# basecomplextech/spec

Hardware: AMD Instinct MI355X
Metric: Mmsg/s + GB/s decode (device-resident), 1M×256B batch, 1/2/4/8 MI355X (higher is better)
Workload: dtype u8; 1 GPU; flat16-decode; records_per_gpu=1048576, stream_bytes_per_gpu=267602339, parallelism=record-sharded x1, no collective, ranks=1, distinct_devices=1, rehearsal=False

## Files before the change

__graft_entry__.py:

```python
from __future__ import annotations

import os
import subprocess
import sys

ROOT = os.path.dirname(os.path.abspath(__file__))


def build() -> None:
    jobs = str(min(8, os.cpu_count() or 1))
    subprocess.run(["make", "-s", "-j", jobs, "-C", os.path.join(ROOT, "spec_amd", "csrc")], check=True)
    subprocess.run(["make", "-s", "-C", os.path.join(ROOT, "oracle")], check=True)
    if ROOT not in sys.path:
        sys.path.insert(0, ROOT)
    import spec_amd

    L = spec_amd.lib()
    import time

    t0 = time.time() - 1
    import ctypes as C

    L.spec_decode_flat_jit_compile(C.byref(spec_amd.FLAT16.c), 1 << 28, 1 << 20)
    from spec_amd import workload

    for sc in workload.bench_wide_schemas().values():
        L.spec_decode_flat_jit_compile(C.byref(sc.c), 1 << 28, 1 << 20)
    L.spec_decode_flat_jit_compile(C.byref(spec_amd.NESTED.item.c), 1 << 28, 1 << 20)
    L.spec_encode_flat_jit_compile(C.byref(spec_amd.FLAT16.c))
    L.spec_decode_nested_jit_compile(C.byref(spec_amd.NESTED.c))
    L.spec_encode_nested_jit_compile(C.byref(spec_amd.NESTED.c))
    from spec_amd.tree_catalog import precompiled_trees

    k = int(jobs)
    procs = [subprocess.Popen([sys.executable, "-c", f"import __graft_entry__ as g; g._compile_trees({i}, {k})"],
                              cwd=ROOT) for i in range(min(k, len(precompiled_trees())))]
    if any(p.wait() != 0 for p in procs):
        raise RuntimeError("schema-tree kernel compile failed")
    procs = [subprocess.Popen([sys.executable, "-c", f"import __graft_entry__ as g; g._compile_sweep({i}, {k})"],
                              cwd=ROOT) for i in range(k)]
    if any(p.wait() != 0 for p in procs):
        raise RuntimeError("shape-sweep kernel compile failed")
    cache = os.path.join(ROOT, "spec_amd", "jit_cache")
    for f in os.listdir(cache):
        if f.endswith(".co") and os.path.getmtime(os.path.join(cache, f)) < t0:
            os.remove(os.path.join(cache, f))


def _compile_trees(i: int, k: int) -> None:
    import ctypes as C

    import spec_amd
    from spec_amd.tree_catalog import precompiled_trees

    L = spec_amd.lib()
    for t in precompiled_trees()[i::k]:
        if L.spec_tree_jit_compile(C.byref(t.c)) <= 0:
            raise RuntimeError("schema-tree kernel compile failed")


def _compile_sweep(i: int, k: int) -> None:
    import ctypes as C

    import spec_amd
    from spec_amd import workload

    L = spec_amd.lib()
    sweep = workload.shape_sweep_schemas()
    work = [(2 if len(s) <= 9 else 24 if len(s) <= 25 else 58, name, "encode") for name, s in sweep.items() if len(s) <= 32]
    work += [(8, name, "decode") for name in sweep]
    shares = [[0, []] for _ in range(k)]
    for cost, name, prog in sorted(work, reverse=True):
        share = min(shares, key=lambda sh: sh[0])
        share[0] += cost
        share[1].append((name, prog))
    for name, prog in shares[i][1]:
        c = C.byref(sweep[name].c)
        size = L.spec_encode_flat_jit_compile(c) if prog == "encode" else L.spec_decode_flat_jit_compile(c, 1 << 28, 1 << 20)
        if size <= 0:
# ... 43 lines not shown
```

spec_amd/csrc/decode_core.hpp:

```cpp
#pragma once

#include "spec_device.hpp"

namespace spec {


struct FieldSet {
    uint8_t *status;
    uint64_t *errmask;
    uint64_t *present;
    uint32_t nfields;
    uint16_t tags[SPEC_KFIELDS];
    uint8_t kinds[SPEC_KFIELDS];
    uint16_t rank[SPEC_KFIELDS];
    void *cols[SPEC_KFIELDS];
};

struct DecodeArgs {
    const uint8_t *stream;
    uint64_t stream_len;
    const uint64_t *ends;
    uint64_t n;
    uint64_t r0;
    uint32_t head;
    uint32_t slab;
    uint32_t xcd;
    FieldSet f;
};

struct NestedArgs {
    const uint8_t *stream;
    uint64_t stream_len;
    const uint64_t *ends;
    uint64_t n;
    FieldSet outer;
    FieldSet item;
    uint32_t list_tag, list_rank;
    uint32_t *item_begin;
    uint64_t item_cap;
    uint64_t *group_base;
    uint64_t *total;
    uint32_t slab;
    uint32_t xcd;
    uint32_t head;
};

constexpr int DEC_WAVES = 4;
constexpr int SLAB_GUARD = 48;

constexpr int SLAB_MAX_CHUNKS = 40;
__host__ __device__ inline uint32_t decode_slab_bytes(double avg_record, double margin = 1.04) {
    const double span = avg_record * 64 * margin;
    int chunks = (int)(span / 1024.0) + 1;
    if (chunks > SLAB_MAX_CHUNKS) return 0;
    return (uint32_t)(SLAB_GUARD + chunks * 1024 + 32);
}
constexpr uint32_t NESTED_SLAB_MAX = 163840 / DEC_WAVES - 1024;
__host__ __device__ inline uint32_t nested_slab_bytes(double avg_record) {
    const uint32_t s = decode_slab_bytes(avg_record, 1.16);
    return s <= NESTED_SLAB_MAX ? s : 0u;
}


template <class Src>
__device__ __noinline__ long long table_search(const Src s, typename Src::pos_t tstart, uint32_t nent,
                                               bool big, uint32_t tag) {
    int left = 0, right = (int)nent - 1;
    while (left <= right) {
        int mid = (int)((unsigned)(left + right) >> 1);
        uint32_t cur;
        typename Src::pos_t p;
        if (big) {
            p = tstart + (typename Src::pos_t)mid * 6;
            cur = (s.u8(p) << 8) | s.u8(p + 1);
        } else {
            p = tstart + (typename Src::pos_t)mid * 3;
            cur = s.u8(p);
        }
        if (cur < tag) {
            left = mid + 1;
        } else if (cur > tag) {
            right = mid - 1;
        } else {
            if (big)
                return ((long long)s.u8(p + 2) << 24) | (s.u8(p + 3) << 16) | (s.u8(p + 4) << 8) | s.u8(p + 5);
            return (s.u8(p + 1) << 8) | s.u8(p + 2);
        }
    }
    return -1;
}


struct Val {
    uint64_t v0, v1, v2, v3;
};

struct Win {
    Tail t;
    uint64_t x0, x1, x2;
};

template <uint32_t KIND>
__host__ __device__ constexpr bool narrow_kind() {
    return KIND == K_BOOL || KIND == K_BYTE || KIND == K_INT16 || KIND == K_INT32 || KIND == K_UINT16 ||
// ... 248 lines not shown

template <bool LIST = false, class Src>
__device__ __forceinline__ Trailer parse_trailer(const Src &s, typename Src::pos_t rs, typename Src::pos_t re) {
    Trailer tr = {ST_OK, false, 0, 0, 0, 0};
    long long len = (long long)(re - rs);
    Tail t = load_tail(s, re);
    uint32_t type = (uint32_t)t.q0 & 0xff;
    const uint32_t T_SMALL = LIST ? T_LIST : T_MESSAGE, T_BIG = LIST ? T_BIG_LIST : T_BIG_MESSAGE;
    const uint32_t ESMALL = LIST ? 2u : 3u, EBIG = LIST ? 4u : 6u;
    if (type != T_SMALL && type != T_BIG) {
        tr.st = ST_INVALID_TYPE;
        return tr;
    }
    tr.big = type == T_BIG;
    uint64_t R = tail_r(t);
    uint32_t R2 = tail_r2(t);
    int m1, m2;
    uint32_t tsz = (uint32_t)rvarint<5>(R, R2, len - 1, m1);
    if (m1 < 0) {
        tr.st = ST_INVALID_TABLE_SIZE;
        return tr;
    }
    uint64_t Rs = (R >> (8 * m1)) | ((uint64_t)R2 << (64 - 8 * m1));
    uint32_t R2s = m1 >= 2 ? 0u : (R2 >> (8 * m1));
    uint32_t dsz = (uint32_t)rvarint<5>(Rs, R2s, len - 1 - m1, m2);
    if (m2 < 0) {
        tr.st = ST_INVALID_DATA_SIZE;
        return tr;
    }
    long long tend = (long long)(re - 1) - m1 - m2;
    long long ts = tend - (long long)tsz;
    if (ts < (long long)rs || tsz % (tr.big ? EBIG : ESMALL) != 0) {
        tr.st = ST_INVALID_TABLE;
        return tr;
    }
    if (ts - (long long)dsz < (long long)rs) {
        tr.st = ST_INVALID_DATA;
        return tr;
    }
    tr.tstart = ts;
    tr.dstart = ts - (long long)dsz;
    tr.dsize = dsz;
    tr.tsize = tsz;
    return tr;
}


struct RecInfo {
    Trailer tr;
    bool ok, sorted;
    uint32_t nent;
};

template <class Src>
__device__ __forceinline__ RecInfo rec_open(const Src &s, typename Src::pos_t rs, typename Src::pos_t re) {
    using pos_t = typename Src::pos_t;
    RecInfo ri;
    ri.tr = Trailer{ST_OK, false, 0, 0, 0, 0};
    ri.ok = false;
    ri.sorted = true;
    ri.nent = 0;
    if (re > rs) {
        ri.tr = parse_trailer(s, rs, re);
        ri.ok = ri.tr.st == ST_OK;
        ri.nent = ri.tr.tsize / (ri.tr.big ? 6u : 3u);
    }
    if (ri.ok) {
        const pos_t tstart = (pos_t)ri.tr.tstart;
        const uint32_t esz = ri.tr.big ? 6u : 3u;
        uint32_t prev = 0;
        bool sorted = true;
        for (uint32_t i0 = 0; i0 < ri.nent; i0 += 8) {
            uint32_t tg[8];
#pragma unroll
            for (int u = 0; u < 8; u++) {
                const uint32_t i = i0 + u < ri.nent ? i0 + u : ri.nent - 1;
                const pos_t p = tstart + (pos_t)(i * esz);
                const uint32_t b0 = s.u8(p), b1 = s.u8(p + 1);
                tg[u] = ri.tr.big ? ((b0 << 8) | b1) : b0;
            }
#pragma unroll
            for (int u = 0; u < 8; u++) {
                const uint32_t i = i0 + u;
                const bool in = i < ri.nent;
                sorted = sorted & !(in & (i > 0) & (tg[u] <= prev));
                prev = in ? tg[u] : prev;
            }
        }
        ri.sorted = sorted;
    }
    return ri;
}

template <class Src>
__device__ __forceinline__ long long rec_field_end(const Src &s, const RecInfo &ri, uint32_t tag, uint32_t k) {
    using pos_t = typename Src::pos_t;
    if (!ri.ok) return -1;
    const pos_t tstart = (pos_t)ri.tr.tstart;
    long long end = -1;
    bool hit = false;
    if (ri.sorted && k < ri.nent) {
        if (ri.tr.big) {
            pos_t p = tstart + (pos_t)k * 6;
            uint32_t tg = (s.u8(p) << 8) | s.u8(p + 1);
            if (tg == tag) {
                end = ((long long)s.u8(p + 2) << 24) | (s.u8(p + 3) << 16) | (s.u8(p + 4) << 8) | s.u8(p + 5);
                hit = true;
            }
        } else {
            pos_t p = tstart + (pos_t)k * 3;
            if (s.u8(p) == tag) {
                end = (s.u8(p + 1) << 8) | s.u8(p + 2);
                hit = true;
            }
        }
    }
    if (!hit) end = table_search(s, tstart, ri.nent, ri.tr.big, tag);
    if (end > (long long)ri.tr.dsize) end = -1;
    return end;
}

template <bool PRESENT = false, class Src>
__device__ __forceinline__ void decode_record_generic(const Src &s, typename Src::pos_t rs, typename Src::pos_t re,
                                                      uint64_t r, const FieldSet &fs, long long to_stream) {
    using pos_t = typename Src::pos_t;
    const RecInfo ri = rec_open(s, rs, re);
    if (fs.status) fs.status[r] = (uint8_t)ri.tr.st;
    const pos_t dstart = (pos_t)ri.tr.dstart;
    uint64_t errs = 0, pres = 0;
    for (uint32_t f = 0; f < fs.nfields; f++) {
        const uint32_t kind = fs.kinds[f];
        if (kind == K_LIST) continue;
        const long long end = rec_field_end(s, ri, fs.tags[f], fs.rank[f]);
        const bool ok = decode_store(s, kind, dstart, end, to_stream, fs.cols[f], r);
        if (!ok && f < 64) errs |= 1ull << f;
        if constexpr (PRESENT) pres |= (end >= 0 && f < 64) ? 1ull << f : 0ull;
    }
    if (fs.errmask) fs.errmask[r] = errs;
    if constexpr (PRESENT) fs.present[r] = pres;
}


struct RuntimeSpec {
    static constexpr int N = 0;
    static constexpr bool big = false;
};

constexpr int FAST_MAX_FIELDS = 24;

template <class Spec>
struct FastRec {
    Win w[Spec::N];
    int e[Spec::N], lo[Spec::N];
};

template <class Spec, int F>
struct FieldLoad {
    static __device__ __forceinline__ void run(FastRec<Spec> &fr, const LdsSrc &s, int ds, const uint32_t *ends,
                                               uint32_t dsize) {
        if constexpr (F < Spec::N) {
            constexpr uint32_t K = Spec::kind[F];
            const uint32_t end = ends[Spec::rank[F]];
            const bool has = (end <= dsize) & (end > 0);
            if constexpr (K == K_LIST) {
                fr.lo[F] = ds;
                fr.e[F] = has ? ds + (int)end : ds;
            } else {
                fr.e[F] = has ? ds + (int)end : SLAB_GUARD;
                fr.lo[F] = has ? ds : SLAB_GUARD;
                fr.w[F] = load_win<K, true>(s, fr.e[F]);
            }
            FieldLoad<Spec, F + 1>::run(fr, s, ds, ends, dsize);
        }
    }
// ... 90 lines not shown
    FieldLoad<Spec, 0>::run(fr, s, (int)tr.dstart, ends, tr.dsize);
    return FieldNat<Spec, 0>::ok(fr);
}

template <class Spec, bool ERR = false>
__device__ __forceinline__ void fast_finish(const FastRec<Spec> &fr, uint64_t r, const FieldSet &fs,
                                            long long to_stream) {
    uint64_t errs = 0;
    FieldStore<Spec, 0, ERR>::run(fr, to_stream, fs, r, errs);
    if (fs.status) fs.status[r] = ST_OK;
    if constexpr (ERR) fs.errmask[r] = errs;
}

constexpr int FAST_BATCH = 8;

template <class Spec, int J0, int K, int NB>
struct WideField {
    static __device__ __forceinline__ void load(Win (&w)[NB], int (&e)[NB], int (&lo)[NB], const LdsSrc &s, int ds,
                                                const uint32_t (&ends)[NB], uint32_t dsize) {
        if constexpr (K < NB) {
            constexpr uint32_t KD = Spec::kind[Spec::order[J0 + K]];
            const bool has = (ends[K] <= dsize) & (ends[K] > 0);
            e[K] = has ? ds + (int)ends[K] : SLAB_GUARD;
            lo[K] = has ? ds : SLAB_GUARD;
            w[K] = load_win<KD, true>(s, e[K]);
            WideField<Spec, J0, K + 1, NB>::load(w, e, lo, s, ds, ends, dsize);
        }
    }
    static __device__ __forceinline__ bool nat(const Win (&w)[NB], const int (&e)[NB], const int (&lo)[NB]) {
        if constexpr (K >= NB) {
            return true;
        } else {
            constexpr uint32_t NT = cross_kind_type(Spec::kind[Spec::order[J0 + K]]);
            bool good = true;
            if constexpr (NT != 0) good = (e[K] <= lo[K]) | (((uint32_t)w[K].t.q0 & 0xff) == NT);
            return good & WideField<Spec, J0, K + 1, NB>::nat(w, e, lo);
        }
    }
    template <bool ERR>
    static __device__ __forceinline__ void store(const Win (&w)[NB], const int (&e)[NB], const int (&lo)[NB],
                                                 long long to_stream, const FieldSet &fs, uint64_t r, uint64_t &errs) {
        if constexpr (K < NB) {
            constexpr int F = Spec::order[J0 + K];
            constexpr uint32_t KD = Spec::kind[F];
            bool ok = true;
            const Val v = decode_tail_k<KD, true>(w[K], lo[K], e[K], to_stream, ERR ? &ok : nullptr);
            store_value_k<KD>(fs.cols[F], r, v);
            if constexpr (ERR && F < 64) errs |= (!ok & (e[K] > lo[K])) ? (1ull << F) : 0ull;
            WideField<Spec, J0, K + 1, NB>::template store<ERR>(w, e, lo, to_stream, fs, r, errs);
        }
    }
};

struct RecMasks {
    uint64_t errs = 0, pres = 0;
};

template <class Spec, int J0, int J1, bool ERR, bool PRESENT = false>
__device__ __forceinline__ bool wide_batch(const LdsSrc &s, int ts, int ds, uint32_t dsize, uint64_t r,
                                           const FieldSet &fs, long long to_stream, RecMasks &m) {
    constexpr int NB = J1 - J0;
    constexpr int ESZ = Spec::big ? 6 : 3;
    constexpr int NC = (ESZ * NB + 7) / 8, NQ = NC + 1;
    const int p0 = ts + ESZ * J0;
    const int base = p0 & ~7;
    const uint32_t sh = 8u * (uint32_t)(p0 & 7);
    uint64_t q[NQ];
#pragma unroll
    for (int j = 0; j < NQ; j++) q[j] = s.d64(base + 8 * j);
    uint64_t c[NC];
#pragma unroll
    for (int j = 0; j < NC; j++) c[j] = (q[j] >> sh) | ((q[j + 1] << 1) << (63 - sh));
    auto byte_at = [&](int j) -> uint32_t { return (uint32_t)(c[j >> 3] >> (8 * (j & 7))) & 0xff; };
    bool hit = true;
    uint32_t ends[NB];
#pragma unroll
    for (int k = 0; k < NB; k++) {
        if constexpr (Spec::big) {
            hit = hit & (((byte_at(6 * k) << 8) | byte_at(6 * k + 1)) == Spec::stag[J0 + k]);
            ends[k] = (byte_at(6 * k + 2) << 24) | (byte_at(6 * k + 3) << 16) | (byte_at(6 * k + 4) << 8) |
                      byte_at(6 * k + 5);
        } else {
            hit = hit & (byte_at(3 * k) == Spec::stag[J0 + k]);
            ends[k] = (byte_at(3 * k + 1) << 8) | byte_at(3 * k + 2);
        }
    }
    if (!hit) return false;
    if constexpr (PRESENT) {
#pragma unroll
        for (int k = 0; k < NB; k++) m.pres |= ends[k] <= dsize ? 1ull << Spec::order[J0 + k] : 0ull;
    }
    Win w[NB];
    int e[NB], lo[NB];
    WideField<Spec, J0, 0, NB>::load(w, e, lo, s, ds, ends, dsize);
    if (!WideField<Spec, J0, 0, NB>::nat(w, e, lo)) return false;
    WideField<Spec, J0, 0, NB>::template store<ERR>(w, e, lo, to_stream, fs, r, m.errs);
    return true;
}


template <class Spec>
struct TagSet {
    static constexpr uint64_t word(int w) {
        uint64_t v = 0;
        for (int k = 0; k < Spec::N; k++)
            if ((int)(Spec::stag[k] >> 6) == w) v |= 1ull << (Spec::stag[k] & 63);
        return v;
    }
};

// ... 40 lines not shown
        ends[k] = has ? end : ~0u;
        m.pres |= (has & (end <= dsize)) ? 1ull << Spec::order[J0 + k] : 0ull;
    }
    Win w[NB];
    int e[NB], lo[NB];
    WideField<Spec, J0, 0, NB>::load(w, e, lo, s, ds, ends, dsize);
    if (!WideField<Spec, J0, 0, NB>::nat(w, e, lo)) return false;
    WideField<Spec, J0, 0, NB>::template store<ERR>(w, e, lo, to_stream, fs, r, m.errs);
    return true;
}

template <class Spec, int J0, int JE, bool ERR>
struct PresentBatchesTo {
    static __device__ __forceinline__ bool run(const LdsSrc &s, int ts, int ds, uint32_t dsize, uint32_t ranks,
                                               uint64_t r, const FieldSet &fs, long long to_stream, RecMasks &m) {
        if constexpr (J0 >= JE) {
            return true;
        } else {
            constexpr int J1 = J0 + FAST_BATCH < JE ? J0 + FAST_BATCH : JE;
            if (!present_batch<Spec, J0, J1, ERR>(s, ts, ds, dsize, ranks, r, fs, to_stream, m)) return false;
            return PresentBatchesTo<Spec, J1, JE, ERR>::run(s, ts, ds, dsize, ranks, r, fs, to_stream, m);
        }
    }
};

template <class Spec, int J0, bool ERR>
struct WideBatches {
    static __device__ __forceinline__ bool run(const LdsSrc &s, int ts, int ds, uint32_t dsize, uint64_t r,
                                               const FieldSet &fs, long long to_stream, RecMasks &m) {
        if constexpr (J0 >= Spec::N) {
            return true;
        } else {
            constexpr int J1 = J0 + FAST_BATCH < Spec::N ? J0 + FAST_BATCH : Spec::N;
            if (!wide_batch<Spec, J0, J1, ERR>(s, ts, ds, dsize, r, fs, to_stream, m)) return false;
            return WideBatches<Spec, J1, ERR>::run(s, ts, ds, dsize, r, fs, to_stream, m);
        }
    }
};

template <class Spec, int J0, int JE, bool ERR = false, bool PRESENT = false>
struct WideBatchesTo {
    static __device__ __forceinline__ bool run(const LdsSrc &s, int ts, int ds, uint32_t dsize, uint64_t r,
                                               const FieldSet &fs, long long to_stream, RecMasks &m) {
        if constexpr (J0 >= JE) {
            return true;
        } else {
            constexpr int J1 = J0 + FAST_BATCH < JE ? J0 + FAST_BATCH : JE;
            if (!wide_batch<Spec, J0, J1, ERR, PRESENT>(s, ts, ds, dsize, r, fs, to_stream, m)) return false;
            return WideBatchesTo<Spec, J1, JE, ERR, PRESENT>::run(s, ts, ds, dsize, r, fs, to_stream, m);
        }
    }
};

template <class Spec, int P>
__host__ __device__ constexpr int flat_part_lo(int h) {
    if (h >= P) return Spec::N;
    if (P == 2) {
        const int mid = ((Spec::N / 2 + FAST_BATCH - 1) / FAST_BATCH) * FAST_BATCH;
        return h == 0 ? 0 : (mid < Spec::N ? mid : Spec::N);
    }
    return (h * Spec::N) / P;
}
template <class Spec, bool ERR, int P, bool PRESENT = false, int H = 0>
__device__ __forceinline__ bool wide_part_run(const LdsSrc &s, const Trailer &tr, uint64_t r, const FieldSet &fs,
                                              long long to_stream, int h, RecMasks &m) {
    if constexpr (H >= P) {
        return true;
    } else {
        constexpr int J0 = flat_part_lo<Spec, P>(H), J1 = flat_part_lo<Spec, P>(H + 1);
        if (h == H)
            return WideBatchesTo<Spec, J0, J1, ERR, PRESENT>::run(s, (int)tr.tstart, (int)tr.dstart, tr.dsize, r, fs,
                                                                  to_stream, m);
        return wide_part_run<Spec, ERR, P, PRESENT, H + 1>(s, tr, r, fs, to_stream, h, m);
    }
}
template <class Spec, bool ERR = false, int P = 2, bool PRESENT = false>
__device__ __forceinline__ bool fast_wide_half(const LdsSrc &s, int rs, int re, uint64_t r, const FieldSet &fs,
                                               long long to_stream, int h, RecMasks &m) {
    if (re <= rs) return false;
    const Trailer tr = parse_trailer(s, rs, re);
    if ((tr.st != ST_OK) | (tr.big != Spec::big) | (tr.tsize != (Spec::big ? 6u : 3u) * (uint32_t)Spec::N)) return false;
    return wide_part_run<Spec, ERR, P, PRESENT>(s, tr, r, fs, to_stream, h, m);
}

template <class Spec, bool ERR, int P, int H = 0>
__device__ __forceinline__ bool present_part_run(const LdsSrc &s, const Trailer &tr, uint32_t ranks, uint64_t r,
                                                 const FieldSet &fs, long long to_stream, int h, RecMasks &m) {
    if constexpr (H >= P) {
        return true;
    } else {
        constexpr int J0 = flat_part_lo<Spec, P>(H), J1 = flat_part_lo<Spec, P>(H + 1);
        if (h == H)
            return PresentBatchesTo<Spec, J0, J1, ERR>::run(s, (int)tr.tstart, (int)tr.dstart, tr.dsize, ranks, r, fs,
                                                            to_stream, m);
        return present_part_run<Spec, ERR, P, H + 1>(s, tr, ranks, r, fs, to_stream, h, m);
    }
}
template <class Spec, bool ERR = false, int P = 2>
__device__ __forceinline__ bool fast_present_half(const LdsSrc &s, int rs, int re, uint64_t r, const FieldSet &fs,
                                                  long long to_stream, int h, RecMasks &m) {
    if (re <= rs) return false;
    const Trailer tr = parse_trailer(s, rs, re);
    if ((tr.st != ST_OK) | tr.big | (tr.tsize > 3u * (uint32_t)Spec::N)) return false;
    uint32_t ranks;
    if (!present_ranks<Spec>(s, (int)tr.tstart, tr.tsize / 3u, ranks)) return false;
    return present_part_run<Spec, ERR, P>(s, tr, ranks, r, fs, to_stream, h, m);
}

template <class Spec, bool ERR = false>
__device__ __forceinline__ bool fast_wide(const LdsSrc &s, int rs, int re, uint64_t r, const FieldSet &fs,
                                          long long to_stream) {
    if (re <= rs) return false;
    const Trailer tr = parse_trailer(s, rs, re);
    if ((tr.st != ST_OK) | (tr.big != Spec::big) | (tr.tsize != (Spec::big ? 6u : 3u) * (uint32_t)Spec::N)) return false;
    RecMasks m;
// ... 41 lines not shown
        __builtin_amdgcn_wave_barrier();
        __builtin_amdgcn_fence(__ATOMIC_ACQUIRE, "wavefront");
    }
}

template <int AUX>
__device__ __forceinline__ void stage_span(__amdgpu_buffer_rsrc_t rsrc, uint8_t *dst, const Staged &st,
                                           uint64_t stream_len, int lane, int part = 0, int parts = 1) {
    stage_issue<AUX>(rsrc, dst, st, lane, part, parts);
    asm volatile("s_waitcnt vmcnt(0)" ::: "memory");
    stage_fix_tail(rsrc, dst, st, stream_len, lane, part, parts);
}

struct Group {
    uint64_t rec_lo, rec_hi;
    Staged st;
    bool in_lds;
    __device__ __forceinline__ int rs() const { return SLAB_GUARD + (int)(rec_lo - st.origin); }
    __device__ __forceinline__ int re() const { return SLAB_GUARD + (int)(rec_hi - st.origin); }
    __device__ __forceinline__ long long to_stream() const { return (long long)st.origin - SLAB_GUARD; }
};

__device__ __forceinline__ uint64_t uniform64(uint64_t v) {
    return __builtin_amdgcn_readfirstlane((uint32_t)v) |
           ((uint64_t)__builtin_amdgcn_readfirstlane((uint32_t)(v >> 32)) << 32);
}

__device__ __forceinline__ void load_group_ends(const DecodeArgs &a, uint64_t base, int lane, uint64_t &lo,
                                                uint64_t &hi) {
    const uint64_t r = base + lane;
    const uint64_t last = a.n - 1;
    hi = a.ends[r < last ? r : last];
    lo = (r == 0 ? 0 : a.ends[(r - 1) < last ? r - 1 : last]) + a.head;
}

__device__ __forceinline__ Group make_group(uint64_t n, uint64_t base, uint64_t lo, uint64_t hi, uint32_t slab,
                                            int l0 = 0, int l1 = 64) {
    Group gr;
    gr.rec_lo = lo;
    gr.rec_hi = hi < lo ? lo : hi;
    const int nrec = (int)(n - base < 64 ? n - base : 64);
    const int last = (l1 < nrec ? l1 : nrec) - 1;
    const uint64_t span_lo = uniform64(__shfl(lo, l0));
    const uint64_t span_hi = uniform64(__shfl(hi, last < 0 ? 0 : last));
    gr.st = stage_plan(span_lo, span_hi);
    gr.in_lds = slab > 0 && l0 <= last && span_hi >= span_lo && SLAB_GUARD + (uint64_t)gr.st.bytes() + 16 <= (uint64_t)slab;
    return gr;
}
__device__ __forceinline__ Group make_group(const DecodeArgs &a, uint64_t base, int lane, uint64_t lo, uint64_t hi,
                                            uint32_t slab) {
    return make_group(a.n, base, lo, hi, slab);
}

template <class Spec, bool ERR = false, bool PRESENT = false>
__device__ __forceinline__ void decode_flat_once(const DecodeArgs &a) {
    static_assert(!PRESENT || Spec::N == 0, "the schema-specialised PRESENT kernel is decode_flat_pair");
    extern __shared__ __attribute__((aligned(16))) uint8_t smem[];
    const int wave = threadIdx.x >> 6;
    const int lane = threadIdx.x & 63;
    uint64_t blk = blockIdx.x;
    if (a.xcd) {
        const uint64_t per = (gridDim.x + 7) / 8;
        blk = (blockIdx.x & 7) * per + (blockIdx.x >> 3);
    }
    const uint64_t base = a.r0 + (blk * (blockDim.x >> 6) + wave) * 64;
    if (base >= a.n) return;
    const uint64_t r = base + lane;
    const bool valid = r < a.n;
    uint8_t *slab = smem + wave * a.slab;
    __amdgpu_buffer_rsrc_t rsrc =
        uniform_rsrc(a.stream, a.stream_len);
    const uint64_t hi = a.ends[valid ? r : a.n - 1];
    uint64_t lo = __shfl_up(hi, 1);
    if (lane == 0) lo = r == 0 ? 0 : a.ends[r - 1];
    lo += a.head;
    const Group cur = make_group(a, base, lane, lo, hi, a.slab);
    if (cur.in_lds) {
        stage_span<STREAM_AUX>(rsrc, slab + SLAB_GUARD, cur.st, a.stream_len, lane);
        if (!valid) return;
        LdsSrc s{(lds_u8 *)slab};
        const int rs = cur.rs(), re = cur.re();
        const long long to_stream = cur.to_stream();
        if constexpr (Spec::N > 0) {
            if constexpr (Spec::N <= FAST_MAX_FIELDS && !Spec::big) {
                FastRec<Spec> fr;
                if (fast_prepare<Spec>(s, rs, re, fr)) {
                    fast_finish<Spec, ERR>(fr, r, a.f, to_stream);
                    return;
                }
            } else {
                if (fast_wide<Spec, ERR>(s, rs, re, r, a.f, to_stream)) return;
            }
        }
        decode_record_generic<PRESENT>(s, rs, re, r, a.f, to_stream);
    } else if (valid) {
        GlobalSrc s{a.stream, a.stream_len};
        decode_record_generic<PRESENT>(s, (long long)cur.rec_lo, (long long)cur.rec_hi, r, a.f, 0);
    }
}

template <class Spec, bool ERR = false, int P = 2, bool PRESENT = false>
__device__ __forceinline__ void decode_flat_pair(const DecodeArgs &a) {
    extern __shared__ __attribute__((aligned(16))) uint8_t smem[];
    const int wave = threadIdx.x >> 6;
    const int lane = threadIdx.x & 63;
    uint64_t blk = blockIdx.x;
    if (a.xcd) {
        const uint64_t per = (gridDim.x + 7) / 8;
        blk = (blockIdx.x & 7) * per + (blockIdx.x >> 3);
    }
    const uint64_t base = a.r0 + blk * 64;
    if (base >= a.n) return;
    const uint64_t r = base + lane;
    const bool valid = r < a.n;
    uint8_t *slab = smem;
    uint32_t *xch = (uint32_t *)(smem + a.slab);
    __amdgpu_buffer_rsrc_t rsrc = uniform_rsrc(a.stream, a.stream_len);
    const uint64_t hi = a.ends[valid ? r : a.n - 1];
    uint64_t lo = __shfl_up(hi, 1);
    if (lane == 0) lo = r == 0 ? 0 : a.ends[r - 1];
    lo += a.head;
    const Group cur = make_group(a, base, lane, lo, hi, a.slab);
    if (!cur.in_lds) {
        if (wave == 0 && valid) {
            GlobalSrc s{a.stream, a.stream_len};
            decode_record_generic<PRESENT>(s, (long long)cur.rec_lo, (long long)cur.rec_hi, r, a.f, 0);
        }
        return;
    }
    stage_span<STREAM_AUX>(rsrc, slab + SLAB_GUARD, cur.st, a.stream_len, lane, wave, P);
    __syncthreads();
    LdsSrc s{(lds_u8 *)slab};
    const int rs = cur.rs(), re = cur.re();
    const long long to_stream = cur.to_stream();
    RecMasks mine;
    bool ok;
    if constexpr (PRESENT && Spec::N <= FAST_MAX_FIELDS && !Spec::big)
        ok = valid && fast_present_half<Spec, ERR, P>(s, rs, re, r, a.f, to_stream, wave, mine);
    else
        ok = valid && fast_wide_half<Spec, ERR, P, PRESENT>(s, rs, re, r, a.f, to_stream, wave, mine);
    uint64_t *xerr = (uint64_t *)(xch + 64 * (P - 1));
    uint64_t *xpres = xerr + (ERR ? 64 * (P - 1) : 0);
    if (wave > 0) {
        xch[64 * (wave - 1) + lane] = ok ? 1u : 0u;
        if constexpr (ERR) xerr[64 * (wave - 1) + lane] = mine.errs;
        if constexpr (PRESENT) xpres[64 * (wave - 1) + lane] = mine.pres;
    }
    __syncthreads();
    if (wave == 0 && valid) {
        bool all = ok;
        uint64_t m = mine.errs, pm = mine.pres;
#pragma unroll
        for (int w = 1; w < P; w++) {
            all = all && xch[64 * (w - 1) + lane] != 0;
            if constexpr (ERR) m |= xerr[64 * (w - 1) + lane];
            if constexpr (PRESENT) pm |= xpres[64 * (w - 1) + lane];
        }
        if (all) {
            if (a.f.status) a.f.status[r] = ST_OK;
            if constexpr (ERR) a.f.errmask[r] = m;
            if constexpr (PRESENT) a.f.present[r] = pm;
        } else {
            decode_record_generic<PRESENT>(s, rs, re, r, a.f, to_stream);
        }
    }
}

struct DecodeLaunch {
    uint32_t slab;
    unsigned blocks;
};

__host__ inline DecodeLaunch decode_launch(uint64_t nrec, double avg_record) {
    DecodeLaunch L;
    L.slab = decode_slab_bytes(avg_record);
    L.blocks = (unsigned)(((nrec + 63) / 64 + 7) / 8 * 8);
    return L;
}

}
```

spec_amd/csrc/decode_flat.hip:

```cpp
#include <hip/hip_runtime.h>

#include "decode_core.hpp"
#include "spec_internal.hpp"

namespace spec {

__global__ __launch_bounds__(256) void decode_flat_kernel(DecodeArgs a) { decode_flat_once<RuntimeSpec>(a); }

__global__ __launch_bounds__(256) void decode_flat_present_kernel(DecodeArgs a) {
    decode_flat_once<RuntimeSpec, false, true>(a);
}

int device_cus() {
    static int cus[64] = {0};
    int dev = 0;
    if (hipGetDevice(&dev) != hipSuccess || dev < 0 || dev >= 64) return 256;
    if (!cus[dev]) {
        int v = 0;
        if (hipDeviceGetAttribute(&v, hipDeviceAttributeMultiprocessorCount, dev) != hipSuccess || v <= 0) v = 256;
        cus[dev] = v;
    }
    return cus[dev];
}

int launch_decode_flat(DecodeArgs a, double avg_record, hipStream_t stream) {
    if (a.n <= a.r0) return 0;
    const DecodeLaunch L = decode_launch(a.n - a.r0, avg_record);
    a.slab = L.slab;
    a.xcd = 1;
    if (a.f.present) hipLaunchKernelGGL(decode_flat_present_kernel, dim3(L.blocks), dim3(64), L.slab, stream, a);
    else hipLaunchKernelGGL(decode_flat_kernel, dim3(L.blocks), dim3(64), L.slab, stream, a);
    return hipGetLastError() == hipSuccess ? 0 : -1;
}

}
```

spec_amd/csrc/jit.cpp:

```cpp
#include <sstream>
#include <string>
#include <vector>
#include <cstring>

#include "jit_module.hpp"
#include "spec_internal.hpp"

namespace {

using namespace spec::jit;

enum DecodeFn { DEC_PAIR, DEC_PAIR_ERR, DEC_PAIR_PRESENT, DEC_PAIR_PRESENT_ERR };
enum EncodeFn { ENC_SIZE, ENC_WRITE, ENC_WRITE_FRAMES };
enum NestedFn { NEST_PAIR, NEST_RANGES };
enum NestedEncFn { NENC_SIZE, NENC_WRITE, NENC_WRITE_FRAMES, NENC_WRITE_PAIR, NENC_WRITE_PAIR_FRAMES };

bool schema_fits(const spec_schema *s, uint32_t max_fields, bool lists, uint32_t max_tag) {
    if (s->nfields == 0 || s->nfields > max_fields) return false;
    for (uint32_t f = 0; !lists && f < s->nfields; f++)
        if (s->fields[f].kind == SPEC_KIND_LIST) return false;
    uint8_t order[SPEC_KFIELDS];
    if (max_tag) spec::table_order(s, order);
    for (uint32_t k = 0, below = 0; max_tag && k < s->nfields; k++) {
        const uint32_t tag = s->fields[order[k]].tag;
// ... 181 lines not shown
    h.e = e;
    return e;
}

bool has_nested_fast_path(const spec_nested_schema *s) {
    return !nested_wide(s) && (has_fast_path(&s->outer) || has_fast_path(&s->item));
}

const Module *lookup_nested(const spec_nested_schema *s, Prog p) {
    if (!enabled() || !(p == NESTED ? has_nested_fast_path(s) : has_nested_encoder(s))) return nullptr;
    int dev = 0;
    if (hipGetDevice(&dev) != hipSuccess) return nullptr;
    const std::string k = key_of(&s->outer, dev, p) + "|" + key_of(&s->item, dev, p) + (p == NESTED ? "" : "|n");
    return find_module(k, p, [&] {
        return load_module(compile_source(p == NESTED ? generate_nested(s) : generate_nested_encode(s), p),
                           nested_kernels(p));
    });
}

}

namespace spec {

long long jit_compile_only(const spec_schema *s, double) {
    return compile_only(has_flat_fast_path(s), DECODE, [&] { return generate_decode(s); });
}
long long jit_compile_only_encode(const spec_schema *s) {
    return compile_only(has_encoder(s), ENCODE, [&] { return generate_encode(s); });
}
long long jit_compile_only_nested(const spec_nested_schema *s) {
    return compile_only(has_nested_fast_path(s), NESTED, [&] { return generate_nested(s); });
}
long long jit_compile_only_nested_encode(const spec_nested_schema *s) {
    return compile_only(has_nested_encoder(s), NESTED_ENC, [&] { return generate_nested_encode(s); });
}

int jit_prepare_decode_flat(const spec_schema *schema, double avg_record) {
    return decode_slab_bytes(avg_record) != 0 && lookup(schema, DECODE) ? 1 : 0;
}

int jit_prepare_encode_flat(const spec_schema *schema) { return lookup(schema, ENCODE) ? 1 : 0; }

int jit_launch_decode_flat(const spec_schema *schema, const DecodeArgs &a, double avg_record, hipStream_t stream) {
    if (decode_slab_bytes(avg_record) == 0) return 0;
    const Module *m = lookup(schema, DECODE);
    if (!m) return 0;
    if (a.n <= a.r0) return 1;
    DecodeArgs args = a;
    args.slab = decode_slab_bytes(avg_record);
    args.xcd = 1;
    const uint64_t groups = ((a.n - a.r0 + 63) / 64 + 7) / 8 * 8;
    const int fn = a.f.present ? (a.f.errmask ? DEC_PAIR_PRESENT_ERR : DEC_PAIR_PRESENT)
                               : (a.f.errmask ? DEC_PAIR_ERR : DEC_PAIR);
    const unsigned xch = 256 + (a.f.errmask ? 512 : 0) + (a.f.present ? 512 : 0);
    return launch_module(m->fn[fn], (unsigned)groups, 64 * FLAT_WAVES, args.slab + (FLAT_WAVES - 1) * xch, stream, &args,
                         sizeof args);
}

int jit_launch_encode(const spec_schema *schema, const EncodeArgs &a, bool write, hipStream_t stream) {
    const Module *m = lookup(schema, ENCODE);
    if (!m) return 0;
    const int fn = !write ? ENC_SIZE : a.frame_head ? ENC_WRITE_FRAMES : ENC_WRITE;
    return launch_module(m->fn[fn], (unsigned)a.nblocks, ENC_BLOCK, write ? (unsigned)enc_write_lds_bytes() : 0, stream, &a,
                         sizeof a);
}

int jit_launch_nested(const spec_nested_schema *schema, const NestedArgs &a, int mode, hipStream_t stream) {
    if (a.slab == 0) return 0;
    const Module *m = lookup_nested(schema, NESTED);
    if (!m) return 0;
    unsigned grid = (unsigned)((a.n + 63) / 64);
    if (a.xcd) grid = (grid + 7) / 8 * 8;
    const bool ranges = mode == NESTED_RANGES;
    const size_t lds = a.slab + (ranges ? NESTED_RANGE_BYTES : 1024u);
    return launch_module(m->fn[ranges ? NEST_RANGES : NEST_PAIR], grid, ranges ? 64 : 64 * NESTED_WAVES, (unsigned)lds,
                         stream, &a, sizeof a);
}

int jit_launch_nested_encode(const spec_nested_schema *schema, const NestedEncodeArgs &a, bool write,
                             hipStream_t stream) {
    const Module *m = lookup_nested(schema, NESTED_ENC);
    if (!m) return 0;
    NestedEncodeArgs args = a;
    args.xcd = write ? 1u : 0u;
    const unsigned lds = (unsigned)(write ? nenc_write_lds_bytes() : nenc_size_lds_bytes());
    const unsigned grid = (unsigned)(args.xcd ? (a.nblocks + 7) / 8 * 8 : a.nblocks);
    const bool pair = write && m->fn[NENC_WRITE_PAIR] && a.item_pre && a.wave_ok;
    const int fn = !write         ? NENC_SIZE
                   : a.frame_head ? (pair ? NENC_WRITE_PAIR_FRAMES : NENC_WRITE_FRAMES)
                                  : (pair ? NENC_WRITE_PAIR : NENC_WRITE);
    return launch_module(m->fn[fn], grid, pair ? 2 * NENC_BLOCK : NENC_BLOCK, lds, stream, &args, sizeof args);
}

}
```

spec_amd/workload.py:

```python
from __future__ import annotations

import numpy as np

from .schema import FLAT16, Kind, Schema

SEED = 0x5EC0DE


def _signed(rng, n, width):
    k = rng.integers(0, width, size=n)
    mag = (rng.integers(0, 2**62, size=n, dtype=np.uint64) << np.uint64(2)) | rng.integers(0, 4, size=n, dtype=np.uint64)
    mask = np.where(k >= 64, np.uint64(~np.uint64(0)), (np.uint64(1) << k.astype(np.uint64)) - np.uint64(1))
    mag &= mask
    v = mag.astype(np.int64)
    neg = rng.integers(0, 2, size=n).astype(bool)
    v = np.where(neg, -v, v)
    return v


def _unsigned(rng, n, width):
    k = rng.integers(0, width + 1, size=n)
    v = (rng.integers(0, 2**62, size=n, dtype=np.uint64) << np.uint64(2)) | rng.integers(0, 4, size=n, dtype=np.uint64)
    shift = np.clip(k, 0, 63).astype(np.uint64)
    mask = np.where(k >= 64, np.uint64(~np.uint64(0)), (np.uint64(1) << shift) - np.uint64(1))
# ... 161 lines not shown
                cols[c.name] = np.where(sp[:, 1] > 0, h[last], 0).astype(np.uint8).reshape(R, 1)
            elif c.role == ROLE_PRESENT:
                cols[c.name] = ((rng.random(R) < present) & live).astype(np.uint8).reshape(R, 1)
            elif c.kind == Kind.ANY:
                a, h = _any_values(rng, R)
                a.view(np.uint32)[~live] = 0
                cols[c.name], heaps[c.name] = a, h
            else:
                a, h = _values(rng, c.kind, R, str_len)
                a[~live] = 0
                cols[c.name] = np.ascontiguousarray(a)
                if h is not None:
                    heaps[c.name] = h if h.size else np.zeros(1, np.uint8)
    return cols, heaps, rows


def bench_wide_schemas():
    from .schema import Kind, Schema

    kinds = [Kind(k) for k in range(1, 16)]
    tags40 = [int(t) for t in np.random.default_rng(3).permutation(np.arange(1, 41))]
    return {"wide40": Schema([(t, kinds[i % 15]) for i, t in enumerate(tags40)]),
            "big16": Schema([(256 + 37 * i, kinds[i % 15]) for i in range(16)])}


def shape_sweep_schemas():
    kinds = [Kind(k) for k in range(1, 16)]

    def cyc(tags, perm_seed=None):
        n = len(tags)
        if perm_seed is not None:
            tags = [int(t) for t in np.random.default_rng(perm_seed).permutation(tags)]
        return Schema([(t, kinds[(15 - n % 15 + i) % 15]) for i, t in enumerate(tags)])

    out = {}
    permuted = {17, 21, 24, 34, 63}
    for n in (1, 2, 8, 9, 17, 18, 21, 22, 24, 25, 32, 33, 34, 49, 63, 64):
        p = n in permuted
        out[f"n{n}{'p' if p else ''}"] = cyc(list(range(1, n + 1)), 100 + n if p else None)
    out["big21"] = cyc([250 + 3 * i for i in range(21)])
    out["big22"] = cyc([250 + 3 * i for i in range(22)])
    out["tag255"] = cyc([254, 255])
    out["tag256"] = cyc([255, 256])
    words = [int(t) for t in np.random.default_rng(8).permutation([1, 63, 64, 127, 128, 191, 192, 255])]
    out["tagwords8"] = Schema(list(zip(words, [Kind.INT32, Kind.STRING, Kind.UINT64, Kind.BYTES, Kind.BOOL,
                                               Kind.FLOAT64, Kind.BIN128, Kind.INT16])))
    out["tags3w"] = cyc([1, 2, 200])
    S, B = Kind.STRING, Kind.BYTES
    out["heap16"] = Schema(list(enumerate([S, B, Kind.INT32, S, B, S, B, Kind.UINT64, S, B, S, B, Kind.INT16, S, B,
                                           Kind.INT64], start=1)))
    return out


LZ4_KINDS = ("text", "random", "mixed", "zeros", "period3", "period200", "records", "chunks", "longlit")


def lz4_chunks(rng, n, lit, rep):
    out = bytearray()
    while len(out) < n:
        out += rng.integers(0, 256, lit, dtype=np.uint8).tobytes()
        src = int(rng.integers(0, max(1, len(out) - rep)))
        out += out[src:src + rep]
    return np.frombuffer(bytes(out[:n]), np.uint8)


def lz4_data(kind: str, n: int) -> np.ndarray:
    rng = np.random.default_rng(sum(kind.encode()) % 1000)
    d = {
        "text": lambda: np.frombuffer((b"spec message field table trailer " * (n // 33 + 1))[:n], np.uint8),
        "random": lambda: rng.integers(0, 256, n, dtype=np.uint8),
        "mixed": lambda: np.concatenate([rng.integers(0, 6, n // 2, dtype=np.uint8),
                                         rng.integers(0, 256, n - n // 2, dtype=np.uint8)]),
        "zeros": lambda: np.zeros(n, np.uint8),
        "period3": lambda: np.frombuffer((b"abc" * (n // 3 + 1))[:n], np.uint8),
        "period200": lambda: np.tile(rng.integers(0, 256, 200, dtype=np.uint8), n // 200 + 1)[:n],
        "records": lambda: np.tile(np.frombuffer(b"".join(bytes([7, i % 13, 0, 0]) + rng.integers(0, 256, 9, dtype=np.uint8)
                                                          .tobytes() for i in range(64)), np.uint8), n // 832 + 1)[:n],
        "chunks": lambda: lz4_chunks(rng, n, 300, 700),
        "longlit": lambda: lz4_chunks(rng, n, 9000, 3000),
    }[kind]()
    return np.ascontiguousarray(d).copy()
```

Measured before the change: 16130 Mmsg/s.

## Pack cross-wave error/present masks and split generic decode fields across waves

The JIT pair decode kernel now packs each wave's ok flag together with its error and present bits into a single 32- or 64-bit word, using the field span that wave owns. This shrinks the LDS exchange area so more blocks can fit per CU; a static assert checks that nine Flat16 error slabs fit. The generic runtime decode kernel is changed from one wave per 64 records to four waves sharing one slab, each wave decoding a subset of fields and merging masks through LDS. This adds __syncthreads and changes the generic path's occupancy profile.

```diff
diff --git a/__graft_entry__.py b/__graft_entry__.py
--- a/__graft_entry__.py
+++ b/__graft_entry__.py
@@ -25,6 +25,8 @@
     from spec_amd import workload
 
     for sc in workload.bench_wide_schemas().values():
+        L.spec_decode_flat_jit_compile(C.byref(sc.c), 1 << 28, 1 << 20)
+    for sc in workload.exchange_limit_schemas().values():
         L.spec_decode_flat_jit_compile(C.byref(sc.c), 1 << 28, 1 << 20)
     L.spec_decode_flat_jit_compile(C.byref(spec_amd.NESTED.item.c), 1 << 28, 1 << 20)
     L.spec_encode_flat_jit_compile(C.byref(spec_amd.FLAT16.c))
diff --git a/spec_amd/csrc/decode_core.hpp b/spec_amd/csrc/decode_core.hpp
--- a/spec_amd/csrc/decode_core.hpp
+++ b/spec_amd/csrc/decode_core.hpp
@@ -49,7 +49,7 @@
 constexpr int SLAB_GUARD = 48;
 
 constexpr int SLAB_MAX_CHUNKS = 40;
-__host__ __device__ inline uint32_t decode_slab_bytes(double avg_record, double margin = 1.04) {
+__host__ __device__ constexpr uint32_t decode_slab_bytes(double avg_record, double margin = 1.04) {
     const double span = avg_record * 64 * margin;
     int chunks = (int)(span / 1024.0) + 1;
     if (chunks > SLAB_MAX_CHUNKS) return 0;
@@ -404,6 +404,7 @@
     uint32_t nent;
 };
 
+
 template <class Src>
 __device__ __forceinline__ RecInfo rec_open(const Src &s, typename Src::pos_t rs, typename Src::pos_t re) {
     using pos_t = typename Src::pos_t;
@@ -472,6 +473,27 @@
     return end;
 }
 
+struct RecMasks {
+    uint64_t errs = 0, pres = 0;
+};
+
+template <bool PRESENT = false, class Src>
+__device__ __forceinline__ RecMasks decode_fields_generic(const Src &s, const RecInfo &ri, uint64_t r, const FieldSet &fs,
+                                                          long long to_stream, uint32_t f_lo, uint32_t f_hi) {
+    using pos_t = typename Src::pos_t;
+    const pos_t dstart = (pos_t)ri.tr.dstart;
+    uint64_t errs = 0, pres = 0;
+    for (uint32_t f = f_lo; f < f_hi; f++) {
+        const uint32_t kind = fs.kinds[f];
+        if (kind == K_LIST) continue;
+        const long long end = rec_field_end(s, ri, fs.tags[f], fs.rank[f]);
+        const bool ok = decode_store(s, kind, dstart, end, to_stream, fs.cols[f], r);
+        if (!ok && f < 64) errs |= 1ull << f;
+        if constexpr (PRESENT) pres |= (end >= 0 && f < 64) ? 1ull << f : 0ull;
+    }
+    return RecMasks{errs, pres};
+}
+
 template <bool PRESENT = false, class Src>
 __device__ __forceinline__ void decode_record_generic(const Src &s, typename Src::pos_t rs, typename Src::pos_t re,
                                                       uint64_t r, const FieldSet &fs, long long to_stream) {
@@ -668,10 +690,6 @@
     }
 };
 
-struct RecMasks {
-    uint64_t errs = 0, pres = 0;
-};
-
 template <class Spec, int J0, int J1, bool ERR, bool PRESENT = false>
 __device__ __forceinline__ bool wide_batch(const LdsSrc &s, int ts, int ds, uint32_t dsize, uint64_t r,
                                            const FieldSet &fs, long long to_stream, RecMasks &m) {
@@ -818,15 +836,55 @@
     }
 };
 
+__host__ __device__ constexpr int flat_part_lo_of(int N, int P, int h) {
+    if (h >= P) return N;
+    if (P == 2) {
+        const int mid = ((N / 2 + FAST_BATCH - 1) / FAST_BATCH) * FAST_BATCH;
+        return h == 0 ? 0 : (mid < N ? mid : N);
+    }
+    return (h * N) / P;
+}
 template <class Spec, int P>
 __host__ __device__ constexpr int flat_part_lo(int h) {
-    if (h >= P) return Spec::N;
-    if (P == 2) {
-        const int mid = ((Spec::N / 2 + FAST_BATCH - 1) / FAST_BATCH) * FAST_BATCH;
-        return h == 0 ? 0 : (mid < Spec::N ? mid : Spec::N);
-    }
-    return (h * Spec::N) / P;
-}
+    return flat_part_lo_of(Spec::N, P, h);
+}
+
+struct PartSpan {
+    int first, width;
+};
+template <class Order>
+__host__ __device__ constexpr PartSpan flat_part_span(const Order *order, int N, int P, int w) {
+    const int j0 = flat_part_lo_of(N, P, w), j1 = flat_part_lo_of(N, P, w + 1);
+    if (j1 <= j0) return PartSpan{0, 0};
+    int lo = (int)order[j0], hi = (int)order[j0];
+    for (int j = j0; j < j1; j++) {
+        lo = (int)order[j] < lo ? (int)order[j] : lo;
+        hi = (int)order[j] > hi ? (int)order[j] : hi;
+    }
+    return PartSpan{lo, hi - lo + 1};
+}
+template <class Order>
+__host__ __device__ constexpr int flat_mask_width(const Order *order, int N, int P) {
+    int width = 0;
+    for (int w = 1; w < P; w++) {
+        const int ww = flat_part_span(order, N, P, w).width;
+        width = ww > width ? ww : width;
+    }
+    return width;
+}
+enum : int { XCH_WORD = 1, XCH_PAIR = 2, XCH_UNPACKED = 0 };
+__host__ __device__ constexpr int flat_exchange_mode(int width, bool err, bool present) {
+    const int bits = 1 + width * ((err ? 1 : 0) + (present ? 1 : 0));
+    return bits <= 32 ? XCH_WORD : bits <= 64 ? XCH_PAIR : XCH_UNPACKED;
+}
+__host__ __device__ constexpr uint32_t flat_exchange_bytes(int P, int width, bool err, bool present) {
+    const int mode = flat_exchange_mode(width, err, present);
+    const uint32_t per = mode == XCH_WORD ? 256u : mode == XCH_PAIR ? 512u : 256u + (err ? 512u : 0u) + (present ? 512u : 0u);
+    return (uint32_t)(P - 1) * per;
+}
+static_assert(flat_exchange_bytes(2, 8, true, false) == flat_exchange_bytes(2, 0, false, false) &&
+                  decode_slab_bytes(255.2) + flat_exchange_bytes(2, 8, true, false) <= 163840 / 9,
+              "nine Flat16 err slabs per CU");
 template <class Spec, bool ERR, int P, bool PRESENT = false, int H = 0>
 __device__ __forceinline__ bool wide_part_run(const LdsSrc &s, const Trailer &tr, uint64_t r, const FieldSet &fs,
                                               long long to_stream, int h, RecMasks &m) {
@@ -974,9 +1032,15 @@
     return make_group(a.n, base, lo, hi, slab);
 }
 
-template <class Spec, bool ERR = false, bool PRESENT = false>
-__device__ __forceinline__ void decode_flat_once(const DecodeArgs &a) {
-    static_assert(!PRESENT || Spec::N == 0, "the schema-specialised PRESENT kernel is decode_flat_pair");
+constexpr int GENERIC_WAVES = 4;
+
+__host__ __device__ constexpr uint32_t generic_exchange_bytes(bool err, bool present) {
+    return (uint32_t)(GENERIC_WAVES - 1) * 512u * ((err ? 1u : 0u) + (present ? 1u : 0u));
+}
+
+template <bool PRESENT = false>
+__device__ __forceinline__ void decode_flat_group(const DecodeArgs &a) {
+    constexpr int P = GENERIC_WAVES;
     extern __shared__ __attribute__((aligned(16))) uint8_t smem[];
     const int wave = threadIdx.x >> 6;
     const int lane = threadIdx.x & 63;
@@ -985,39 +1049,52 @@
         const uint64_t per = (gridDim.x + 7) / 8;
         blk = (blockIdx.x & 7) * per + (blockIdx.x >> 3);
     }
-    const uint64_t base = a.r0 + (blk * (blockDim.x >> 6) + wave) * 64;
+    const uint64_t base = a.r0 + blk * 64;
     if (base >= a.n) return;
     const uint64_t r = base + lane;
     const bool valid = r < a.n;
-    uint8_t *slab = smem + wave * a.slab;
-    __amdgpu_buffer_rsrc_t rsrc =
-        uniform_rsrc(a.stream, a.stream_len);
+    uint8_t *slab = smem;
+    uint64_t *xerr = (uint64_t *)(smem + a.slab);
+    uint64_t *xpres = xerr + (a.f.errmask ? 64 * (P - 1) : 0);
+    __amdgpu_buffer_rsrc_t rsrc = uniform_rsrc(a.stream, a.stream_len);
     const uint64_t hi = a.ends[valid ? r : a.n - 1];
     uint64_t lo = __shfl_up(hi, 1);
     if (lane == 0) lo = r == 0 ? 0 : a.ends[r - 1];
     lo += a.head;
     const Group cur = make_group(a, base, lane, lo, hi, a.slab);
+    const uint32_t f_lo = ((uint32_t)wave * a.f.nfields) / P, f_hi = ((uint32_t)(wave + 1) * a.f.nfields) / P;
+    RecMasks mine;
     if (cur.in_lds) {
-        stage_span<STREAM_AUX>(rsrc, slab + SLAB_GUARD, cur.st, a.stream_len, lane);
-        if (!valid) return;
-        LdsSrc s{(lds_u8 *)slab};
-        const int rs = cur.rs(), re = cur.re();
-        const long long to_stream = cur.to_stream();
-        if constexpr (Spec::N > 0) {
-            if constexpr (Spec::N <= FAST_MAX_FIELDS && !Spec::big) {
-                FastRec<Spec> fr;
-                if (fast_prepare<Spec>(s, rs, re, fr)) {
-                    fast_finish<Spec, ERR>(fr, r, a.f, to_stream);
-                    return;
-                }
-            } else {
-                if (fast_wide<Spec, ERR>(s, rs, re, r, a.f, to_stream)) return;
-            }
-        }
-        decode_record_generic<PRESENT>(s, rs, re, r, a.f, to_stream);
+        stage_span<STREAM_AUX>(rsrc, slab + SLAB_GUARD, cur.st, a.stream_len, lane, wave, P);
+        __syncthreads();
+        if (valid) {
+            LdsSrc s{(lds_u8 *)slab};
+            const RecInfo ri = rec_open(s, cur.rs(), cur.re());
+            if (wave == 0 && a.f.status) a.f.status[r] = (uint8_t)ri.tr.st;
+            mine = decode_fields_generic<PRESENT>(s, ri, r, a.f, cur.to_stream(), f_lo, f_hi);
+        }
     } else if (valid) {
         GlobalSrc s{a.stream, a.stream_len};
-        decode_record_generic<PRESENT>(s, (long long)cur.rec_lo, (long long)cur.rec_hi, r, a.f, 0);
+        const RecInfo ri = rec_open(s, (long long)cur.rec_lo, (long long)cur.rec_hi);
+        if (wave == 0 && a.f.status) a.f.status[r] = (uint8_t)ri.tr.st;
+        mine = decode_fields_generic<PRESENT>(s, ri, r, a.f, 0, f_lo, f_hi);
+    }
+    if (!a.f.errmask && !PRESENT) return;
+    if constexpr (P > 1) {
+        if (wave > 0) {
+            if (a.f.errmask) xerr[64 * (wave - 1) + lane] = mine.errs;
+            if constexpr (PRESENT) xpres[64 * (wave - 1) + lane] = mine.pres;
+        }
+        __syncthreads();
+    }
+    if (wave == 0 && valid) {
+#pragma unroll
+        for (int w = 1; w < P; w++) {
+            if (a.f.errmask) mine.errs |= xerr[64 * (w - 1) + lane];
+            if constexpr (PRESENT) mine.pres |= xpres[64 * (w - 1) + lane];
+        }
+        if (a.f.errmask) a.f.errmask[r] = mine.errs;
+        if constexpr (PRESENT) a.f.present[r] = mine.pres;
     }
 }
 
@@ -1061,12 +1138,28 @@
         ok = valid && fast_present_half<Spec, ERR, P>(s, rs, re, r, a.f, to_stream, wave, mine);
     else
         ok = valid && fast_wide_half<Spec, ERR, P, PRESENT>(s, rs, re, r, a.f, to_stream, wave, mine);
-    uint64_t *xerr = (uint64_t *)(xch + 64 * (P - 1));
-    uint64_t *xpres = xerr + (ERR ? 64 * (P - 1) : 0);
-    if (wave > 0) {
-        xch[64 * (wave - 1) + lane] = ok ? 1u : 0u;
-        if constexpr (ERR) xerr[64 * (wave - 1) + lane] = mine.errs;
-        if constexpr (PRESENT) xpres[64 * (wave - 1) + lane] = mine.pres;
+    constexpr int XW = (ERR || PRESENT) ? flat_mask_width(Spec::order, Spec::N, P) : 0;
+    constexpr int XMODE = flat_exchange_mode(XW, ERR, PRESENT);
+    constexpr int XPRES = 1 + (ERR ? XW : 0);
+    if constexpr (!ERR && !PRESENT) {
+        if (wave > 0) xch[64 * (wave - 1) + lane] = ok ? 1u : 0u;
+    } else if constexpr (XMODE == XCH_UNPACKED) {
+        uint64_t *xerr = (uint64_t *)(xch + 64 * (P - 1));
+        uint64_t *xpres = xerr + (ERR ? 64 * (P - 1) : 0);
+        if (wave > 0) {
+            xch[64 * (wave - 1) + lane] = ok ? 1u : 0u;
+            if constexpr (ERR) xerr[64 * (wave - 1) + lane] = mine.errs;
+            if constexpr (PRESENT) xpres[64 * (wave - 1) + lane] = mine.pres;
+        }
+    } else if (wave > 0) {
+        int first = 0;
+#pragma unroll
+        for (int w = 1; w < P; w++) first = wave == w ? flat_part_span(Spec::order, Spec::N, P, w).first : first;
+        uint64_t pk = ok ? 1u : 0u;
+        if constexpr (ERR) pk |= (mine.errs >> first) << 1;
+        if constexpr (PRESENT) pk |= (mine.pres >> first) << XPRES;
+        if constexpr (XMODE == XCH_WORD) xch[64 * (wave - 1) + lane] = (uint32_t)pk;
+        else ((uint64_t *)xch)[64 * (wave - 1) + lane] = pk;
     }
     __syncthreads();
     if (wave == 0 && valid) {
@@ -1074,9 +1167,23 @@
         uint64_t m = mine.errs, pm = mine.pres;
 #pragma unroll
         for (int w = 1; w < P; w++) {
-            all = all && xch[64 * (w - 1) + lane] != 0;
-            if constexpr (ERR) m |= xerr[64 * (w - 1) + lane];
-            if constexpr (PRESENT) pm |= xpres[64 * (w - 1) + lane];
+            if constexpr (!ERR && !PRESENT) {
+                all = all && xch[64 * (w - 1) + lane] != 0;
+            } else if constexpr (XMODE == XCH_UNPACKED) {
+                const uint64_t *xerr = (const uint64_t *)(xch + 64 * (P - 1));
+                const uint64_t *xpres = xerr + (ERR ? 64 * (P - 1) : 0);
+                all = all && xch[64 * (w - 1) + lane] != 0;
+                if constexpr (ERR) m |= xerr[64 * (w - 1) + lane];
+                if constexpr (PRESENT) pm |= xpres[64 * (w - 1) + lane];
+            } else {
+                const int first = flat_part_span(Spec::order, Spec::N, P, w).first;
+                constexpr uint64_t bits = XW >= 64 ? ~0ull : (1ull << XW) - 1;
+                const uint64_t pk = XMODE == XCH_WORD ? (uint64_t)xch[64 * (w - 1) + lane]
+                                                      : ((const uint64_t *)xch)[64 * (w - 1) + lane];
+                all = all && (pk & 1) != 0;
+                if constexpr (ERR) m |= ((pk >> 1) & bits) << first;
+                if constexpr (PRESENT) pm |= ((pk >> XPRES) & bits) << first;
+            }
         }
         if (all) {
             if (a.f.status) a.f.status[r] = ST_OK;
diff --git a/spec_amd/csrc/decode_flat.hip b/spec_amd/csrc/decode_flat.hip
--- a/spec_amd/csrc/decode_flat.hip
+++ b/spec_amd/csrc/decode_flat.hip
@@ -5,10 +5,10 @@
 
 namespace spec {
 
-__global__ __launch_bounds__(256) void decode_flat_kernel(DecodeArgs a) { decode_flat_once<RuntimeSpec>(a); }
+__global__ __launch_bounds__(64 * GENERIC_WAVES) void decode_flat_kernel(DecodeArgs a) { decode_flat_group<false>(a); }
 
-__global__ __launch_bounds__(256) void decode_flat_present_kernel(DecodeArgs a) {
-    decode_flat_once<RuntimeSpec, false, true>(a);
+__global__ __launch_bounds__(64 * GENERIC_WAVES) void decode_flat_present_kernel(DecodeArgs a) {
+    decode_flat_group<true>(a);
 }
 
 int device_cus() {
@@ -28,8 +28,10 @@
     const DecodeLaunch L = decode_launch(a.n - a.r0, avg_record);
     a.slab = L.slab;
     a.xcd = 1;
-    if (a.f.present) hipLaunchKernelGGL(decode_flat_present_kernel, dim3(L.blocks), dim3(64), L.slab, stream, a);
-    else hipLaunchKernelGGL(decode_flat_kernel, dim3(L.blocks), dim3(64), L.slab, stream, a);
+    const unsigned lds = L.slab + generic_exchange_bytes(a.f.errmask != nullptr, a.f.present != nullptr);
+    const dim3 block(64 * GENERIC_WAVES);
+    if (a.f.present) hipLaunchKernelGGL(decode_flat_present_kernel, dim3(L.blocks), block, lds, stream, a);
+    else hipLaunchKernelGGL(decode_flat_kernel, dim3(L.blocks), block, lds, stream, a);
     return hipGetLastError() == hipSuccess ? 0 : -1;
 }
 
diff --git a/spec_amd/csrc/jit.cpp b/spec_amd/csrc/jit.cpp
--- a/spec_amd/csrc/jit.cpp
+++ b/spec_amd/csrc/jit.cpp
@@ -257,9 +257,14 @@
     const uint64_t groups = ((a.n - a.r0 + 63) / 64 + 7) / 8 * 8;
     const int fn = a.f.present ? (a.f.errmask ? DEC_PAIR_PRESENT_ERR : DEC_PAIR_PRESENT)
                                : (a.f.errmask ? DEC_PAIR_ERR : DEC_PAIR);
-    const unsigned xch = 256 + (a.f.errmask ? 512 : 0) + (a.f.present ? 512 : 0);
-    return launch_module(m->fn[fn], (unsigned)groups, 64 * FLAT_WAVES, args.slab + (FLAT_WAVES - 1) * xch, stream, &args,
-                         sizeof args);
+    int width = 0;
+    if (a.f.errmask || a.f.present) {
+        uint8_t order[SPEC_KFIELDS];
+        table_order(schema, order);
+        width = flat_mask_width(order, (int)schema->nfields, FLAT_WAVES);
+    }
+    const unsigned xch = flat_exchange_bytes(FLAT_WAVES, width, a.f.errmask != nullptr, a.f.present != nullptr);
+    return launch_module(m->fn[fn], (unsigned)groups, 64 * FLAT_WAVES, args.slab + xch, stream, &args, sizeof args);
 }
 
 int jit_launch_encode(const spec_schema *schema, const EncodeArgs &a, bool write, hipStream_t stream) {
diff --git a/spec_amd/workload.py b/spec_amd/workload.py
--- a/spec_amd/workload.py
+++ b/spec_amd/workload.py
@@ -237,6 +237,11 @@
     return out
 
 
+def exchange_limit_schemas():
+    kinds = [Kind(k) for k in range(1, 16)]
+    return {"n31": Schema([(t, kinds[(15 - 31 % 15 + i) % 15]) for i, t in enumerate(range(1, 32))])}
+
+
 LZ4_KINDS = ("text", "random", "mixed", "zeros", "period3", "period200", "records", "chunks", "longlit")
 
 
```

Result: no change. 16120 Mmsg/s (-0.1%).
